# microsoft/AI2BMD

Hardware: NVIDIA H100
Metric: MD steps/sec (higher is better)
Workload: dtype f32

## Files before the change

### ai2bmd_b200/csrc/engine.cu

```cuda
#include <cuda_runtime.h>

#include <algorithm>
#include <cstdarg>
#include <cstdio>
#include <cstdlib>
#include <cstring>
#include <mutex>
#include <string>
#include <vector>

#include "../../include/visnet_b200.h"
#include "k_edge.cuh"
#include "k_caph.cuh"
#include "k_comm.cuh"
#include "k_edge_tc.cuh"
#include "k_graph_embed.cuh"
#include <nvtx3/nvToolsExt.h>
#include "k_head.cuh"
#include "k_md.cuh"
#include "k_nonbonded.cuh"
#include "k_node.cuh"
#include "k_node2.cuh"
#include "k_node_tc.cuh"

// ... 321 lines not shown
        if (status == cudaSuccess && e != cudaSuccess) status = e;
    }
};

template <int NPW>
void launch_head(Launcher& Lc) {
    vb_handle* h = Lc.h;
    const int blocks = (h->ws.N + NODE_WARPS * NPW - 1) / (NODE_WARPS * NPW);
    Lc.launch(head_kernel<NPW>, dim3(blocks), dim3(NODE_WARPS * 32), HeadSmem<NPW>::BYTES, h->mw, h->ws);
    Lc.check();
}
template <int TE, int NW>
void launch_edge_fwd(Launcher& Lc, int l, int occ) {
    vb_handle* h = Lc.h;
    EdgeArgs a{l, h->mw, h->ws};
    const int tiles = (h->ws.Ecap + TE - 1) / TE;
    const int blocks = std::max(1, std::min(tiles, h->sm_count * occ));
    Lc.launch(edge_fwd_kernel<TE, NW>, dim3(blocks), dim3(NW * 32), edge_fwd_smem_bytes<TE>(), a);
    Lc.check();
}
template <int TE, int NW>
void launch_edge_bwd(Launcher& Lc, int l, int occ) {
    vb_handle* h = Lc.h;
    EdgeArgs a{l, h->mw, h->ws};
    const int tiles = (h->ws.Ecap + TE - 1) / TE;
    const int blocks = std::max(1, std::min(tiles, h->sm_count * occ));
    Lc.launch(edge_bwd_kernel<TE, NW>, dim3(blocks), dim3(NW * 32), edge_bwd_smem_bytes<TE>(), a);
    Lc.check();
}

template <int NB>
void launch_node_fwd2(Launcher& Lc, int k) {
    vb_handle* h = Lc.h;
    NodeArgs a{k, h->mw, h->ws, h->timeline ? h->d_tl + (size_t)2 * L * TC_TL_SLOTS + (size_t)k * N2_TL_SLOTS : nullptr, h->krot};
    Lc.launch(node_fwd2_kernel<NB>, dim3((h->ws.N + NB - 1) / NB), dim3(N2Cfg<NB>::THREADS), sizeof(NodeFwd2Smem<NB>), a);
    Lc.check();
}
template <int NB>
void launch_node_bwd2(Launcher& Lc, int k) {
    vb_handle* h = Lc.h;
    NodeArgs a{k, h->mw, h->ws, h->timeline ? h->d_tl + (size_t)2 * L * TC_TL_SLOTS + (size_t)(L + 1 + k) * N2_TL_SLOTS : nullptr, h->krot};
    Lc.launch(node_bwd2_kernel<NB>, dim3((h->ws.N + NB - 1) / NB), dim3(N2Cfg<NB>::THREADS), sizeof(NodeBwd2Smem<NB>), a);
    Lc.check();
}
int node_nb(const vb_handle* h) {
    if (h->node_nb > 0) return h->node_nb;
    for (int nb = 1; nb <= 4; nb++)
        if ((h->ws.N + nb - 1) / nb <= h->sm_count) return nb;
    return 8;
}
void node_fwd(Launcher& Lc, int k) {
    if (Lc.h->npw == 2) launch_node_fwd2<16>(Lc, k);
    else switch (node_nb(Lc.h)) {
        case 1: launch_node_fwd2<1>(Lc, k); break;
        case 2: launch_node_fwd2<2>(Lc, k); break;
        case 3: launch_node_fwd2<3>(Lc, k); break;
        case 4: launch_node_fwd2<4>(Lc, k); break;
        default: launch_node_fwd2<8>(Lc, k);
    }
}
void node_bwd(Launcher& Lc, int k) {
    switch (node_nb(Lc.h)) {
        case 1: launch_node_bwd2<1>(Lc, k); break;
        case 2: launch_node_bwd2<2>(Lc, k); break;
        case 3: launch_node_bwd2<3>(Lc, k); break;
        case 4: launch_node_bwd2<4>(Lc, k); break;
        default: launch_node_bwd2<8>(Lc, k);
    }
}
void head(Launcher& Lc) {
    vb_handle* h = Lc.h;
    if (h->ws.N <= 4096) {
        Lc.launch(head2_kernel, dim3(h->ws.N), dim3(128), 0, h->mw, h->ws);
        Lc.check();
        return;
    }
    h->npw == 2 ? launch_head<2>(Lc) : launch_head<1>(Lc);
}
void launch_edge_fwd_tc(Launcher& Lc, int l) {
    vb_handle* h = Lc.h;
    EdgeTcArgs a{};
    a.layer = l; a.mw = h->mw; a.ws = h->ws;
    const LayerW& lw = h->mw.layer[l];
    const size_t chunk = 4 * 8192;
    int n = 0;
    a.jobs[n++] = TcJob{lw.tcW1, 0};
    a.jobs[n++] = TcJob{lw.tcW1 + chunk, 0};
    if (l < L - 1) a.jobs[n++] = TcJob{lw.tcW1 + 2 * chunk, 0};
    a.jobs[n++] = TcJob{lw.tcWs, 0};
    a.jobs[n++] = TcJob{lw.tcWs + chunk, 0};
    a.njobs = n;
    a.tl = h->timeline ? h->d_tl + (size_t)l * TC_TL_SLOTS : nullptr;
    a.tile_rows = h->tile_rows;
    const int rows = h->tc_rows;
    const int tiles = (h->ws.Ecap + h->tile_rows - 1) / h->tile_rows;
    const int blocks = std::max(1, std::min(tiles, h->sm_count));
    if (rows == 32) Lc.launch(edge_fwd_tc_kernel<32>, dim3(blocks), dim3(TC2_THREADS), TC_SMEM_BYTES, a);
    else if (rows == 64) Lc.launch(edge_fwd_tc_kernel<64>, dim3(blocks), dim3(TC2_THREADS), TC_SMEM_BYTES, a);
    else if (rows == 96) Lc.launch(edge_fwd_tc_kernel<96>, dim3(blocks), dim3(TC2_THREADS), TC_SMEM_BYTES, a);
    else Lc.launch(edge_fwd_tc_kernel<128>, dim3(blocks), dim3(TC2_THREADS), TC_SMEM_BYTES, a);
    Lc.check();
}

void edge_fwd(Launcher& Lc, int l) {
    if (Lc.h->edge_tc & 1) { launch_edge_fwd_tc(Lc, l); return; }
    if (Lc.h->te_fwd == 64) launch_edge_fwd<64, 8>(Lc, l, 2);
    else launch_edge_fwd<32, 8>(Lc, l, 4);
}
void launch_edge_bwd_tc(Launcher& Lc, int l) {
    vb_handle* h = Lc.h;
    EdgeTcArgs a{};
    a.layer = l; a.mw = h->mw; a.ws = h->ws;
    const LayerW& lw = h->mw.layer[l];
    const size_t chunk = 4 * 8192;
    const bool upd = l < L - 1;
    int n = 0;
    a.jobs[n++] = TcJob{lw.tcWsN, 0};
    a.jobs[n++] = TcJob{lw.tcWsN + chunk, 1};
    a.jobs[n++] = TcJob{lw.tcW1N + chunk, 0};
    a.jobs[n++] = TcJob{lw.tcW1N, 1};
    if (upd) a.jobs[n++] = TcJob{lw.tcW1N + 2 * chunk, 1};
    a.njobs = n;
    a.tl = h->timeline ? h->d_tl + (size_t)(L + l) * TC_TL_SLOTS : nullptr;
    a.tile_rows = h->tile_rows;
    const int rows = h->tc_rows;
    const int tiles = (h->ws.Ecap + h->tile_rows - 1) / h->tile_rows;
    const int blocks = std::max(1, std::min(tiles, h->sm_count));
    if (rows == 32) Lc.launch(edge_bwd_tc_kernel<32>, dim3(blocks), dim3(TC2_THREADS), TC_SMEM_BYTES, a);
    else if (rows == 64) Lc.launch(edge_bwd_tc_kernel<64>, dim3(blocks), dim3(TC2_THREADS), TC_SMEM_BYTES, a);
    else if (rows == 96) Lc.launch(edge_bwd_tc_kernel<96>, dim3(blocks), dim3(TC2_THREADS), TC_SMEM_BYTES, a);
    else Lc.launch(edge_bwd_tc_kernel<128>, dim3(blocks), dim3(TC2_THREADS), TC_SMEM_BYTES, a);
    Lc.check();
}

void edge_bwd(Launcher& Lc, int l) {
    if (Lc.h->edge_tc & 2) { launch_edge_bwd_tc(Lc, l); return; }
    if (Lc.h->te_bwd == 64) launch_edge_bwd<64, 8>(Lc, l, 1);
    else launch_edge_bwd<32, 8>(Lc, l, 2);
}

void node_tc_common(const vb_handle* h, NodeTcArgs& a, int k) {
    a.layer = k; a.mw = h->mw; a.ws = h->ws;
    a.tx = (h->ws.N + TC_TE - 1) / TC_TE;
    a.tv = (3 * h->ws.N + TC_TE - 1) / TC_TE;
    a.njx = 3; a.njv = 5; a.jx = 1; a.jv = 1;
}
void node_tc_jobs(TcJob* jobs, const float* img, int n) {
    for (int c = 0; c < n; c++) jobs[c] = TcJob{img + (size_t)c * 4 * 8192, 0};
}
int node_tc_grid(const NodeTcArgs& a) { return a.tx * (a.njx / a.jx) + a.tv * (a.njv / a.jv); }
bool node_tc_split(const vb_handle* h, const NodeTcArgs&) { return h->ws.gxa_parts == 3; }

void launch_node_oproj_tc(Launcher& Lc, int k) {
    vb_handle* h = Lc.h;
    NodeTcArgs a{};
    node_tc_common(h, a, k);
    a.tv = 0;
    node_tc_jobs(a.jobs_x, h->mw.layer[k - 1].tcWo, 3);
    if (!node_tc_split(h, a)) a.jx = 3;
    Lc.launch(node_tc_kernel<NT_OPROJ>, dim3(node_tc_grid(a)), dim3(TC2_THREADS), TC_SMEM_BYTES, a);
    Lc.check();
}
void launch_node_norm_fwd(Launcher& Lc, int k) {
    vb_handle* h = Lc.h;
    Lc.launch(node_norm_fwd_kernel, dim3((h->ws.N + NN_WARPS - 1) / NN_WARPS), dim3(NN_WARPS * 32), 0, k, h->mw, h->ws);
    Lc.check();
}
void launch_node_proj_tc(Launcher& Lc, int k) {
    vb_handle* h = Lc.h;
    NodeTcArgs a{};
    node_tc_common(h, a, k);
    node_tc_jobs(a.jobs_x, h->mw.layer[k].tcWqkv, 3);
    node_tc_jobs(a.jobs_v, h->mw.layer[k].tcWvt, 5);
    if (k == 0) a.tv = 0;
    if (k == L - 1) a.njv = 3;
    if (!node_tc_split(h, a)) { a.jx = a.njx; a.jv = a.njv; }
    Lc.launch(node_tc_kernel<NT_PROJ>, dim3(node_tc_grid(a)), dim3(TC2_THREADS), TC_SMEM_BYTES, a);
    Lc.check();
}
void launch_node_bwdA_tc(Launcher& Lc, int k) {
    vb_handle* h = Lc.h;
    NodeTcArgs a{};
    node_tc_common(h, a, k);
    node_tc_jobs(a.jobs_x, h->mw.layer[k].tcWqkvN, 3);
    node_tc_jobs(a.jobs_v, h->mw.layer[k].tcWvtN, 5);
    if (k == L - 1) a.njv = 3;
    a.acc_qkv = h->ws.GQKV; a.acc_tu = h->ws.GTU;
    if (!node_tc_split(h, a)) { a.jx = a.njx; a.jv = a.njv; }
    Lc.launch(node_tc_kernel<NT_BWDA>, dim3(node_tc_grid(a)), dim3(TC2_THREADS), TC_SMEM_BYTES, a);
    Lc.check();
}
void launch_node_norm_bwd(Launcher& Lc, int k) {
    vb_handle* h = Lc.h;
    NodeTcArgs a{};
    node_tc_common(h, a, k);
    if (k == L - 1) a.njv = 3;
    Lc.launch(node_norm_bwd_kernel, dim3((h->ws.N + NN_WARPS - 1) / NN_WARPS), dim3(NN_WARPS * 32), 0, k, h->mw, h->ws,
              h->ws.GQKV, h->ws.GVNMSG, h->ws.GTU, node_tc_split(h, a) ? 1 : 0);
    Lc.check();
}
void launch_node_bwdB_tc(Launcher& Lc, int k) {
    vb_handle* h = Lc.h;
    NodeTcArgs a{};
    node_tc_common(h, a, k);
    a.tv = 0;
    node_tc_jobs(a.jobs_x, h->mw.layer[k - 1].tcWoN, 3);
    if (h->ws.gxa_parts == 1) a.jx = 3;
    Lc.launch(node_tc_kernel<NT_BWDB>, dim3(node_tc_grid(a)), dim3(TC2_THREADS), TC_SMEM_BYTES, a);
    Lc.check();
}
void node_fwd_tc(Launcher& Lc, int k) {
    char name[64];
    if (k >= 1) { snprintf(name, sizeof(name), "oproj%d", k); if (Lc.next(name)) launch_node_oproj_tc(Lc, k); }
    snprintf(name, sizeof(name), "norm%d", k);
    if (Lc.next(name)) launch_node_norm_fwd(Lc, k);
    if (k < L) { snprintf(name, sizeof(name), "proj%d", k); if (Lc.next(name)) launch_node_proj_tc(Lc, k); }
}
void node_bwd_tc(Launcher& Lc, int k) {
    char name[64];
    if (k <= L - 1) { snprintf(name, sizeof(name), "bwdA%d", k); if (Lc.next(name)) launch_node_bwdA_tc(Lc, k); }
    snprintf(name, sizeof(name), "bnorm%d", k);
    if (Lc.next(name)) launch_node_norm_bwd(Lc, k);
    if (k >= 1) { snprintf(name, sizeof(name), "bwdB%d", k); if (Lc.next(name)) launch_node_bwdB_tc(Lc, k); }
}

void enqueue_finalize(Launcher& Lc, const StepIO& io) {
    vb_handle* h = Lc.h;
    const Workspace& ws = h->ws;
    const bool prot = io.ef != nullptr;
    const int fb = (ws.G + FIN_THREADS / 32 - 1) / (FIN_THREADS / 32);
    const int pb = prot ? (h->n_protein + FIN_THREADS - 1) / FIN_THREADS : 0;
// ... 966 lines not shown
    if (k == "caph_ready") return h->caph_ready ? 1 : 0;
    if (k == "caph_evals") {
        int v = 0;
        if (!h->caph_ready || cudaDeviceSynchronize() != cudaSuccess ||
            cudaMemcpy(&v, h->caph.evals_out, sizeof(int), cudaMemcpyDeviceToHost) != cudaSuccess) return VB_ERR_STATE;
        return v;
    }
    if (k == "comm_ready") return h->comm_ready ? 1 : 0;
    if (k == "edge_overflow") {
        int flag = 0;
        if (h->d_flags && cudaMemcpy(&flag, h->d_flags, sizeof(int), cudaMemcpyDeviceToHost) != cudaSuccess) return VB_ERR_CUDA;
        return flag;
    }
    if (k == "timeline") return h->timeline;
    if (k == "tc_rows") return h->tc_rows;
    if (k == "tile_rows") return h->tile_rows;
    if (k == "n_edges_capacity") return h->ws.Ecap;
    return VB_ERR_ARG;
}

int vb_num_stages(const vb_handle* h) { return h ? (int)h->stage_names.size() : 0; }
const char* vb_stage_name(const vb_handle* h, int stage) {
    if (!h || stage < 0 || stage >= (int)h->stage_names.size()) return "";
    return h->stage_names[stage].c_str();
}

int vb_debug_run(vb_handle* h, const float* pos_dev, int n_stages) {
    if (!h) return VB_ERR_ARG;
    std::lock_guard<std::mutex> lk(h->mu);
    if (!h->has_topology || !pos_dev) { h->set_error("vb_debug_run: bad state/arguments"); return VB_ERR_STATE; }
    CUDA_TRY(h, cudaSetDevice(h->device));
    CUDA_TRY(h, cudaMemcpy(h->d_pos, pos_dev, sizeof(float) * 3 * h->ws.N, cudaMemcpyDeviceToDevice));
    if (h->accum_dirty) { if (int rc = clean_accumulators(h, h->own_stream)) return rc; }
    Launcher Lc{h, h->own_stream, n_stages, 0, false};
    enqueue_all(Lc, internal_io(h, h->n_protein > 0));
    if (Lc.status != cudaSuccess) { h->set_error("debug launch failed: %s", cudaGetErrorString(Lc.status)); return VB_ERR_CUDA; }
    CUDA_TRY(h, cudaStreamSynchronize(h->own_stream));
    h->accum_dirty = n_stages >= 0 && n_stages < (int)h->stage_names.size();
    return VB_OK;
}

int vb_profile_stages(vb_handle* h, const float* pos_dev, int n_iter, float* ms_per_stage_host) {
    if (!h) return VB_ERR_ARG;
    std::lock_guard<std::mutex> lk(h->mu);
    if (!h->has_topology || !pos_dev || !ms_per_stage_host || n_iter <= 0) { h->set_error("vb_profile_stages: bad state/arguments"); return VB_ERR_STATE; }
    CUDA_TRY(h, cudaSetDevice(h->device));
    const int ns = (int)h->stage_names.size();
    std::vector<cudaEvent_t> ev(ns + 1);
    for (auto& e : ev) CUDA_TRY(h, cudaEventCreate(&e));
    std::vector<double> acc(ns, 0.0);
    CUDA_TRY(h, cudaMemcpy(h->d_pos, pos_dev, sizeof(float) * 3 * h->ws.N, cudaMemcpyDeviceToDevice));
    int rc = VB_OK;
    for (int it = 0; it < n_iter + 1 && rc == VB_OK; it++) {
        Launcher Lc{h, h->own_stream, -1, 0, false};
        Lc.events = &ev;
        enqueue_all(Lc, internal_io(h, h->n_protein > 0));
        cudaEventRecord(ev[ns], h->own_stream);
        if (Lc.status != cudaSuccess || cudaStreamSynchronize(h->own_stream) != cudaSuccess) {
            h->set_error("vb_profile_stages: launch failed: %s", cudaGetErrorString(cudaGetLastError()));
            rc = VB_ERR_CUDA;
            break;
        }
        if (it == 0) continue;
        for (int s = 0; s < ns; s++) {
            float ms = 0.f;
            cudaEventElapsedTime(&ms, ev[s], ev[s + 1]);
            acc[s] += ms;
        }
    }
    for (auto& e : ev) cudaEventDestroy(e);
    if (rc == VB_OK)
        for (int s = 0; s < ns; s++) ms_per_stage_host[s] = (float)(acc[s] / n_iter);
    return rc;
}

int vb_tc_selftest(int device, const float* a_host, const float* img_host, float* d_host, int reps, float* ms_out) {
    return vb_tc_selftest_rows(device, TC_TE, a_host, img_host, d_host, reps, ms_out);
}

int vb_tc_selftest_rows(int device, int rows, const float* a_host, const float* img_host, float* d_host, int reps, float* ms_out) {
    if (!a_host || !img_host || !d_host || reps <= 0 || (rows != 32 && rows != 64 && rows != TC_TE)) return VB_ERR_ARG;
    if (cudaSetDevice(device) != cudaSuccess) { g_create_error = "vb_tc_selftest: cudaSetDevice failed"; return VB_ERR_CUDA; }
    float *dA = nullptr, *dI = nullptr, *dD = nullptr;
    const size_t nA = (size_t)TC_TE * D * sizeof(float), nI = (size_t)(D / tc::SLAB_K) * tc::STAGE_BYTES;
    cudaMalloc(&dA, nA); cudaMalloc(&dI, nI); cudaMalloc(&dD, nA);
    cudaMemcpy(dA, a_host, nA, cudaMemcpyHostToDevice);
    cudaMemcpy(dI, img_host, nI, cudaMemcpyHostToDevice);
    cudaMemset(dD, 0, nA);
    void (*kernel)(const float*, const float*, float*, int) =
        rows == 32 ? tc_selftest_kernel<32> : rows == 64 ? tc_selftest_kernel<64> : tc_selftest_kernel<TC_TE>;
    cudaFuncSetAttribute(kernel, cudaFuncAttributeMaxDynamicSharedMemorySize, (int)TC_SMEM_BYTES);
    cudaEvent_t e0, e1;
    cudaEventCreate(&e0); cudaEventCreate(&e1);
    cudaEventRecord(e0);
    kernel<<<1, TC2_THREADS, TC_SMEM_BYTES>>>(dA, dI, dD, reps);
    cudaEventRecord(e1);
    cudaError_t err = cudaDeviceSynchronize();
    float ms = 0.f;
    cudaEventElapsedTime(&ms, e0, e1);
    if (ms_out) *ms_out = ms;
    if (err == cudaSuccess) err = cudaMemcpy(d_host, dD, nA, cudaMemcpyDeviceToHost);
    cudaFree(dA); cudaFree(dI); cudaFree(dD);
    cudaEventDestroy(e0); cudaEventDestroy(e1);
    if (err != cudaSuccess) { g_create_error = std::string("vb_tc_selftest: ") + cudaGetErrorString(err); return VB_ERR_CUDA; }
    return VB_OK;
}

int64_t vb_debug_read(vb_handle* h, const char* name, int layer, void* host_dst, int64_t cap_bytes) {
    if (!h || !name || !host_dst) return VB_ERR_ARG;
    std::lock_guard<std::mutex> lk(h->mu);
    if (!h->has_topology) return VB_ERR_STATE;
    const Workspace& ws = h->ws;
    const size_t N = ws.N, E = ws.Ecap, G = ws.G;
    const void* src = nullptr;
    size_t bytes = 0;
    const std::string k(name);
    auto lay = [&](int hi) { return layer >= 0 && layer < hi; };
#define BUF(key, ptr, count, elt) if (k == key) { src = (ptr); bytes = (size_t)(count) * (elt); }
    if (k == "X" && lay(L + 1)) { src = ws.X[layer]; bytes = N * D * 4; }
    else if (k == "V" && lay(L + 1)) { src = ws.V[layer]; bytes = N * 3 * D * 4; }
    else if (k == "F" && lay(L)) { src = ws.F[layer]; bytes = E * D * 4; }
    else if (k == "VN" && lay(L)) { src = ws.VN[layer]; bytes = N * 3 * D * 4; }
    else if (k == "QKV" && lay(L)) { src = ws.QKV[layer]; bytes = N * 3 * D * 4; }
    else if (k == "V123" && lay(L)) { src = ws.V123[layer]; bytes = N * 9 * D * 4; }
    else if (k == "VDOT" && lay(L)) { src = ws.VDOT[layer]; bytes = N * D * 4; }
    else if (k == "TU" && lay(L)) { src = ws.TU[layer]; bytes = N * 6 * D * 4; }
    else if (k == "O" && lay(L)) { src = ws.O[layer]; bytes = N * 3 * D * 4; }
    else if (k == "P1" && lay(L)) { src = ws.P1[layer]; bytes = E * 3 * D * 4; }
    else if (k == "SP" && lay(L)) { src = ws.SP[layer]; bytes = E * 2 * D * 4; }
    else if (k == "ATT" && lay(L)) { src = ws.ATT[layer]; bytes = E * H * 4; }
    else if (k == "TL" && lay(2 * L) && h->d_tl) { src = h->d_tl + (size_t)layer * TC_TL_SLOTS; bytes = TC_TL_SLOTS * 8; }
    else if (k == "TLN" && lay(2 * L + 3) && h->d_tl) { src = h->d_tl + (size_t)2 * L * TC_TL_SLOTS + (size_t)layer * N2_TL_SLOTS; bytes = N2_TL_SLOTS * 8; }
    else BUF("XA", ws.XA, N * D, 4)
    else BUF("VA", ws.VA, N * 3 * D, 4)
    else BUF("GX", ws.GX, N * D, 4)
    else BUF("GVEC", ws.GVEC, N * 3 * D, 4)
    else BUF("GF", ws.GF, E * D, 4)
    else BUF("GXA", ws.GXA, N * D, 4)
    else BUF("GXA3", ws.GXA, 3 * N * D, 4)
    else BUF("GQKV", ws.GQKV, N * 3 * D, 4)
    else BUF("GVNMSG", ws.GVNMSG, N * 3 * D, 4)
    else BUF("GTU", ws.GTU, N * 6 * D, 4)
    else BUF("geom", ws.geom, E * 8, 4)
    else BUF("rbf", ws.rbf, E * NR, 4)
    else BUF("eacc", ws.eacc, E * 4, 4)
    else BUF("grbf", ws.grbf, E * NR, 4)
    else BUF("esrc", ws.esrc, E, 4)
    else BUF("edst", ws.edst, E, 4)
    else BUF("rowptr", ws.rowptr, N + 1, 4)
    else BUF("eatom", ws.eatom, N, 4)
    else BUF("energy", h->d_energy, G, 4)
    else BUF("forces", h->d_forces, N * 3, 4)
#undef BUF
    if (!src) { h->set_error("vb_debug_read: unknown buffer %s[%d]", name, layer); return VB_ERR_ARG; }
    if ((int64_t)bytes > cap_bytes) bytes = (size_t)cap_bytes;
    if (cudaSetDevice(h->device) != cudaSuccess || cudaDeviceSynchronize() != cudaSuccess ||
        cudaMemcpy(host_dst, src, bytes, cudaMemcpyDeviceToHost) != cudaSuccess) {
        h->set_error("vb_debug_read: copy failed: %s", cudaGetErrorString(cudaGetLastError()));
        return VB_ERR_CUDA;
    }
    return (int64_t)bytes;
}

}
```

### ai2bmd_b200/csrc/k_edge_tc.cuh

```cuda
#pragma once
#include "k_edge.cuh"
#include "tc_common.cuh"

namespace vb {

constexpr int TC_TE = 128;
constexpr int TC_STAGES = 2;
constexpr int TC_MAX_STAGES = 3;
constexpr int TC_SLABS = D / tc::SLAB_K;
static_assert((TC_SLABS & (TC_SLABS - 1)) == 0, "tc_slab rotates the slab order with a mask: TC_SLABS must be a power of two");
constexpr int TC_MAXJOBS = 12;
constexpr int TC_LT = D + LDS_PAD;

struct TcJob {
    const float* img;
    int accumulate;
};

struct TcShared {
    alignas(1024) uint8_t ring[TC_STAGES][tc::STAGE_BYTES];
    alignas(16) float tile[TC_TE][TC_LT];
    alignas(16) float abuf[TC_TE][TC_LT];
    EdgeMeta<TC_TE> meta;
    alignas(8) uint64_t b_full[TC_MAX_STAGES];
    uint64_t b_tile;
    uint32_t released[TC_MAX_STAGES];
    const TcJob* jobs;
    int njobs, nslabs;
    alignas(16) float eacc[TC_TE][4];
    float gattn[TC_TE][H];
};

__device__ __forceinline__ TcShared* tc_shared_base(uint8_t* raw) {
    const uint32_t s = tc::smem_u32(raw);
    return reinterpret_cast<TcShared*>(raw + (((s + 1023u) & ~1023u) - s));
}
constexpr size_t TC_SMEM_BYTES = sizeof(TcShared) + 1024;
static_assert(TC_SMEM_BYTES <= 227 * 1024, "tensor-core kernels must fit the 227 KB of shared memory of an H100 block");

__host__ __device__ constexpr int tc_nstages(int rows) { return rows <= 64 ? 3 : 2; }
constexpr size_t TC_STAGE2_OFF = offsetof(TcShared, abuf) + sizeof(float) * 64 * TC_LT;
static_assert(TC_STAGE2_OFF % 1024 == 0 && sizeof(float) * (TC_TE - 64) * TC_LT >= tc::STAGE_BYTES,
              "the third ring stage must fit the upper half of abuf on a swizzle-atom boundary");
__device__ __forceinline__ uint8_t* tc_stage_ptr(TcShared& sh, int stage) {
    return stage < TC_STAGES ? sh.ring[stage] : reinterpret_cast<uint8_t*>(&sh.abuf[64][0]);
}

__device__ __forceinline__ int tc_slab(int s) { return (s + (int)blockIdx.x) & (TC_SLABS - 1); }

template <int NS>
__device__ __forceinline__ void tc_issue(TcShared& sh, int k) {
    if (k >= sh.nslabs) return;
    const int stage = k % NS, job = (k / TC_SLABS) % sh.njobs, s = tc_slab(k % TC_SLABS);
    const char* src = reinterpret_cast<const char*>(sh.jobs[job].img) + (size_t)s * tc::STAGE_BYTES;
    tc::mbar_arrive_expect_tx(&sh.b_full[stage], tc::STAGE_BYTES);
    tc::tma_load_1d(tc_stage_ptr(sh, stage), src, tc::STAGE_BYTES, &sh.b_full[stage]);
}

}


namespace vb {

constexpr int TC2_CWARPS = 16;
constexpr int TC2_CTHREADS = TC2_CWARPS * 32;
constexpr int TC2_THREADS = TC2_CTHREADS;
constexpr int TC2_NGRP = TC2_CTHREADS / D;

struct EdgeTcArgs {
    int layer;
    ModelW mw;
    Workspace ws;
    TcJob jobs[TC_MAXJOBS];
    int njobs;
    int tile_rows;
    unsigned long long* tl;
};
constexpr int TC_TL_SLOTS = 64;
#define TC_TL(k) do { if (a.tl != nullptr && blockIdx.x == 0 && it == 0 && threadIdx.x == 0) a.tl[k] = (unsigned long long)clock64(); } while (0)

__device__ __forceinline__ void csync() { asm volatile("bar.sync 1, %0;" ::"n"(TC2_CTHREADS) : "memory"); }

template <int ROWS>
struct TcRing {
    static constexpr int NS = tc_nstages(ROWS);
    int next = 0;
};

template <int ROWS>
__device__ __forceinline__ void tc2_setup(TcShared& sh, const TcRing<ROWS>&, const TcJob* jobs, int njobs, int ntiles) {
    constexpr int NS = TcRing<ROWS>::NS;
    if (threadIdx.x == 0) {
        for (int s = 0; s < NS; s++) { tc::mbar_init(&sh.b_full[s], 1); sh.released[s] = 0; }
        tc::mbar_init(&sh.b_tile, TC2_CWARPS);
        sh.jobs = jobs; sh.njobs = njobs; sh.nslabs = ntiles * njobs * TC_SLABS;
        tc::fence_barrier_init();
    }
    __syncthreads();
    if (threadIdx.x == 0)
        for (int k = 0; k < NS; k++) tc_issue<NS>(sh, k);
}

template <int NS>
__device__ __forceinline__ void tc2_release(TcShared& sh, int k, int lane) {
    __syncwarp();
    if (lane == 0) {
        const uint32_t before = tc::atom_add_acq_rel(&sh.released[k % NS], 1u);
        if (before % TC2_CWARPS == TC2_CWARPS - 1) tc_issue<NS>(sh, k + NS);
    }
}

__device__ __forceinline__ void tc2_tile_to_a(TcShared& sh, int rows) {
    csync();
    for (int idx = threadIdx.x; idx < rows * (D / 4); idx += TC2_CTHREADS) {
        const int r = idx >> 5, c = (idx & 31) * 4;
        st4(&sh.abuf[r][c], ld4(&sh.tile[r][c]));
    }
}

template <int ROWS>
__device__ __forceinline__ void tc2_mma(TcShared& sh, TcRing<ROWS>& ring, float (&acc)[32], int accumulate, int warp, int lane,
                                        int nvalid) {
    constexpr int NS = TcRing<ROWS>::NS;
    csync();
    const int q = warp >> 2, m0 = (q & 1) * 64 + (warp & 3) * 16, g = lane >> 2, t = lane & 3;
    const bool active = (q & 1) * 64 < nvalid;
    if (!accumulate) {
#pragma unroll
        for (int i = 0; i < 32; i++) acc[i] = 0.f;
    }
#pragma unroll 1
    for (int s = 0; s < TC_SLABS; s++) {
        const int k = ring.next + s, stage = k % NS;
        if (active) {
            uint32_t ahi[4][4], alo[4][4];
            const int k0 = tc_slab(s) * tc::SLAB_K + t;
#pragma unroll
            for (int kk = 0; kk < 4; kk++) {
                const int kc = k0 + kk * 8;
                tc::split_tf32(sh.abuf[m0 + g][kc], ahi[kk][0], alo[kk][0]);
                tc::split_tf32(sh.abuf[m0 + g + 8][kc], ahi[kk][1], alo[kk][1]);
                tc::split_tf32(sh.abuf[m0 + g][kc + 4], ahi[kk][2], alo[kk][2]);
                tc::split_tf32(sh.abuf[m0 + g + 8][kc + 4], ahi[kk][3], alo[kk][3]);
            }
            tc::mbar_wait(&sh.b_full[stage], (uint32_t)(k / NS) & 1u);
            const uint32_t bhi = tc::smem_u32(tc_stage_ptr(sh, stage)) + (uint32_t)(q >> 1) * (64 * 128);
            const uint32_t blo = bhi + tc::SLAB_BYTES;
            tc::wgmma_fence();
#pragma unroll
            for (int kk = 0; kk < 4; kk++) {
                const uint64_t dhi = tc::smem_desc_sw128(bhi + kk * 32);
                const uint64_t dlo = tc::smem_desc_sw128(blo + kk * 32);
                tc::mma_m64n64k8_tf32(acc, alo[kk], dhi);
                tc::mma_m64n64k8_tf32(acc, ahi[kk], dlo);
                tc::mma_m64n64k8_tf32(acc, ahi[kk], dhi);
            }
            tc::wgmma_commit();
            tc::wgmma_wait_all();
#pragma unroll
            for (int kk = 0; kk < 4; kk++)
#pragma unroll
                for (int i = 0; i < 4; i++) { tc::reg_fence(ahi[kk][i]); tc::reg_fence(alo[kk][i]); }
#pragma unroll
            for (int i = 0; i < 32; i++) tc::reg_fence(acc[i]);
        } else {
            tc::mbar_wait(&sh.b_full[stage], (uint32_t)(k / NS) & 1u);
        }
        tc2_release<NS>(sh, k, lane);
    }
    ring.next += TC_SLABS;
}

__device__ __forceinline__ void tc2_acc_to_tile(TcShared& sh, const float (&acc)[32], int warp, int lane, int nvalid) {
    const int q = warp >> 2, r = (q & 1) * 64 + (warp & 3) * 16 + (lane >> 2), c = (q >> 1) * 64 + 2 * (lane & 3);
#pragma unroll
    for (int i = 0; i < 8; i++) {
        if (r < nvalid) *reinterpret_cast<float2*>(&sh.tile[r][c + 8 * i]) = make_float2(acc[4 * i], acc[4 * i + 1]);
        if (r + 8 < nvalid) *reinterpret_cast<float2*>(&sh.tile[r + 8][c + 8 * i]) = make_float2(acc[4 * i + 2], acc[4 * i + 3]);
    }
}

template <int ROWS>
__global__ void __launch_bounds__(TC2_THREADS, 1) tc_selftest_kernel(const float* __restrict__ A, const float* __restrict__ img,
                                                                     float* __restrict__ Dout, int reps) {
    extern __shared__ __align__(1024) uint8_t dyn_raw[];
    TcShared& sh = *tc_shared_base(dyn_raw);
    __shared__ TcJob jobs[1];
    if (threadIdx.x == 0) jobs[0] = TcJob{img, 0};
    TcRing<ROWS> ring;
    tc2_setup(sh, ring, jobs, 1, reps);
    const int warp = threadIdx.x >> 5, lane = threadIdx.x & 31;
    float acc[32];
    for (int t = 0; t < reps; t++) {
        for (int idx = threadIdx.x; idx < ROWS * (D / 4); idx += TC2_CTHREADS) {
            const int r = idx >> 5, c = (idx & 31) * 4;
            st4(&sh.tile[r][c], ld4(A + (size_t)r * D + c));
        }
        tc2_tile_to_a(sh, ROWS);
        tc2_mma(sh, ring, acc, 0, warp, lane, ROWS);
        csync();
        tc2_acc_to_tile(sh, acc, warp, lane, ROWS);
        csync();
        for (int idx = threadIdx.x; idx < ROWS * (D / 4); idx += TC2_CTHREADS) {
            const int r = idx >> 5, c = (idx & 31) * 4;
            st4(Dout + (size_t)r * D + c, ld4(&sh.tile[r][c]));
        }
        csync();
    }
}

template <int ROWS>
__global__ void __launch_bounds__(TC2_THREADS, 1) edge_fwd_tc_kernel(const __grid_constant__ EdgeTcArgs a) {
    pdl_entry();
    extern __shared__ __align__(1024) uint8_t dyn_raw[];
    TcShared& sh = *tc_shared_base(dyn_raw);
    const Workspace& ws = a.ws;
    const int l = a.layer;
    const LayerW& lw = a.mw.layer[l];
    const bool upd = (l < L - 1);
    const int J_DK = 0, J_DV = 1, J_F = 2, J_S1 = upd ? 3 : 2, J_S2 = upd ? 4 : 3;
    constexpr int RPW = ROWS / TC2_CWARPS;
    const int warp = threadIdx.x >> 5, lane = threadIdx.x & 31, col = lane * 4;
    const int E = ws.rowptr[ws.N];
    const int trows = min(ROWS, max(16, a.tile_rows));
    const int ntiles_total = (E + trows - 1) / trows;
    const int my_tiles = ((int)blockIdx.x < ntiles_total) ? (ntiles_total - (int)blockIdx.x + (int)gridDim.x - 1) / (int)gridDim.x : 0;
    if (a.tl != nullptr && blockIdx.x == 0 && threadIdx.x == 0) a.tl[0] = (unsigned long long)clock64();
    TcRing<ROWS> ring;
// ... 562 lines not shown
```

### ai2bmd_b200/csrc/model.h

```cpp
#pragma once
#include <cuda_runtime.h>
#include <stddef.h>
#include "common.cuh"

namespace vb {

#define VB_GLOBAL_WEIGHTS(X)                                                                      \
    X(emb, 100 * D)                \
    X(nb_emb, 100 * D)             \
    X(rbf_means, NR) X(rbf_betas, NR)                                                              \
    X(WdN, D * NR) X(WdT, NR * D) X(bd, D)      \
    X(WcT, 2 * D * D) X(bc, D) X(WcN, D * 2 * D)         \
    X(WeN, D * NR) X(WeT, NR * D) X(be, D)              \
    X(on_w, D) X(on_b, D) X(von_w, D)          \
    X(h0_W1T, D * D) X(h0_W1N, D * D)                  \
    X(h0_W2T, D * 64) X(h0_W2N, 64 * D)                \
    X(h0_U0T, 2 * D * D) X(h0_b0, D) X(h0_U0N, D * 2 * D)         \
    X(h0_U2T, D * D) X(h0_b2, D) X(h0_U2N, D * D)                 \
    X(h1_W1T, 64 * 64) X(h1_W1N, 64 * 64)              \
    X(h1_U0T, D * 64) X(h1_b0, 64) X(h1_U0N, 64 * D)              \
    X(h1_u2, 64) X(h1_b2, 4)                        \
    X(atomref, 100) X(scalars, 4)

#define VB_LAYER_WEIGHTS(X)                                                                       \
    X(ln_w, D) X(ln_b, D) X(vln_w, D)                                                              \
    X(WqkvT, D * 3 * D) X(bqkv, 3 * D) X(WqkvN, 3 * D * D)           \
    X(WvecT, D * 3 * D) X(WvecN, 3 * D * D)                          \
    X(WtuT, D * 2 * D) X(WtuN, 2 * D * D)                     \
    X(W1T, D * 3 * D) X(b1, 3 * D) X(W1N, 3 * D * D)          \
    X(WsT, D * 2 * D) X(bs, 2 * D) X(WsN, 2 * D * D)                 \
    X(WoT, D * 3 * D) X(bo, 3 * D) X(WoN, 3 * D * D)                 \
     \
    X(tcW1, 3 * 4 * 8192)              \
    X(tcWs, 2 * 4 * 8192)              \
    X(tcWsN, 2 * 4 * 8192)             \
    X(tcW1N, 3 * 4 * 8192)             \
                     \
    X(tcWo, 3 * 4 * 8192)              \
    X(tcWqkv, 3 * 4 * 8192)            \
    X(tcWvt, 5 * 4 * 8192)      \
    X(tcWoN, 3 * 4 * 8192)             \
    X(tcWqkvN, 3 * 4 * 8192)           \
    X(tcWvtN, 5 * 4 * 8192)

struct LayerW {
#define X(name, count) const float* name;
    VB_LAYER_WEIGHTS(X)
#undef X
};

struct ModelW {
#define X(name, count) const float* name;
    VB_GLOBAL_WEIGHTS(X)
#undef X
    LayerW layer[L];
    float cutoff;
};

struct Workspace {
    int N, G, Ecap;
    const int* z;
    const int* frag_of;
    const int* frag_start;
    int* deg;
    int* slots;
    int* rowptr;
    int* esrc;
    int* edst;
    float* geom;
    float* rbf;
    float* eacc;
    float* grbf;
    float* X[L + 1];
    float* V[L + 1];
    float* F[L];
    float* VN[L];
    float* QKV[L];
    float* V123[L];
    float* VDOT[L];
    float* TU[L];
    float* O[L];
    float* P1[L];
    float* SP[L];
    float* ATT[L];
    float* XA;
    float* VA;
    float* GX;
    float* GVEC;
    float* GF;
    float* GXA;
    int gxa_parts;
    float* GQKV;
    float* GVNMSG;
    float* GTU;
    float* eatom;
    float* XN;
    float* PX;
    float* PV;
    float* GO;
};

__device__ __forceinline__ float4 load_gxa(const Workspace& ws, size_t node, int col) {
    float4 v = ld4(ws.GXA + node * D + col);
    if (ws.gxa_parts == 3) v = (v + ld4(ws.GXA + ((size_t)ws.N + node) * D + col)) + ld4(ws.GXA + (2 * (size_t)ws.N + node) * D + col);
    return v;
}

}
```

### ai2bmd_b200/csrc/tc_common.cuh

```cuda
#pragma once
#include <cuda_runtime.h>
#include <stdint.h>

namespace vb {
namespace tc {

__device__ __forceinline__ uint32_t smem_u32(const void* p) { return (uint32_t)__cvta_generic_to_shared(p); }

__device__ __forceinline__ void mbar_init(uint64_t* bar, uint32_t count) {
    asm volatile("mbarrier.init.shared::cta.b64 [%0], %1;" ::"r"(smem_u32(bar)), "r"(count));
}
__device__ __forceinline__ void fence_barrier_init() { asm volatile("fence.mbarrier_init.release.cluster;" ::: "memory"); }
__device__ __forceinline__ void mbar_arrive(uint64_t* bar) {
    asm volatile("{\n\t.reg .b64 st;\n\tmbarrier.arrive.shared::cta.b64 st, [%0];\n\t}" ::"r"(smem_u32(bar)) : "memory");
}
__device__ __forceinline__ void mbar_arrive_expect_tx(uint64_t* bar, uint32_t bytes) {
    asm volatile("{\n\t.reg .b64 st;\n\tmbarrier.arrive.expect_tx.shared::cta.b64 st, [%0], %1;\n\t}" ::"r"(smem_u32(bar)),
                 "r"(bytes)
                 : "memory");
}
__device__ __forceinline__ uint32_t atom_add_acq_rel(uint32_t* p, uint32_t v) {
    uint32_t old;
    asm volatile("atom.acq_rel.cta.shared::cta.add.u32 %0, [%1], %2;" : "=r"(old) : "r"(smem_u32(p)), "r"(v) : "memory");
    return old;
}
__device__ __forceinline__ void mbar_wait(uint64_t* bar, uint32_t parity) {
    asm volatile(
        "{\n\t"
        ".reg .pred p;\n\t"
        "WAIT_LOOP:\n\t"
        "mbarrier.try_wait.parity.shared::cta.b64 p, [%0], %1;\n\t"
        "@p bra WAIT_DONE;\n\t"
        "bra WAIT_LOOP;\n\t"
        "WAIT_DONE:\n\t"
        "}" ::"r"(smem_u32(bar)),
        "r"(parity)
        : "memory");
}

__device__ __forceinline__ void tma_load_1d(void* smem_dst, const void* gmem_src, uint32_t bytes, uint64_t* bar) {
    asm volatile("cp.async.bulk.shared::cluster.global.mbarrier::complete_tx::bytes [%0], [%1], %2, [%3];" ::"r"(
                     smem_u32(smem_dst)),
                 "l"(gmem_src), "r"(bytes), "r"(smem_u32(bar))
                 : "memory");
}

__device__ __forceinline__ void tma_prefetch_l2(const void* gmem_src, uint32_t bytes) {
    asm volatile("cp.async.bulk.prefetch.L2.global [%0], %1;" ::"l"(gmem_src), "r"(bytes) : "memory");
}

__device__ __forceinline__ uint64_t smem_desc_sw128(uint32_t saddr) {
    return (uint64_t)((saddr & 0x3FFFFu) >> 4) | (1ull << 16) | (64ull << 32) | (1ull << 62);
}
__device__ __forceinline__ void wgmma_fence() { asm volatile("wgmma.fence.sync.aligned;" ::: "memory"); }
__device__ __forceinline__ void wgmma_commit() { asm volatile("wgmma.commit_group.sync.aligned;" ::: "memory"); }
__device__ __forceinline__ void wgmma_wait_all() { asm volatile("wgmma.wait_group.sync.aligned 0;" ::: "memory"); }
__device__ __forceinline__ void reg_fence(uint32_t& r) { asm volatile("" : "+r"(r)::"memory"); }
__device__ __forceinline__ void reg_fence(float& r) { asm volatile("" : "+f"(r)::"memory"); }

__device__ __forceinline__ void mma_m64n64k8_tf32(float (&d)[32], const uint32_t (&a)[4], uint64_t desc_b) {
    asm volatile(
        "{\n\t"
        "wgmma.mma_async.sync.aligned.m64n64k8.f32.tf32.tf32 "
        "{%0,%1,%2,%3,%4,%5,%6,%7,%8,%9,%10,%11,%12,%13,%14,%15,"
        "%16,%17,%18,%19,%20,%21,%22,%23,%24,%25,%26,%27,%28,%29,%30,%31}, "
        "{%32,%33,%34,%35}, %36, 1, 1, 1;\n\t"
        "}"
        : "+f"(d[0]), "+f"(d[1]), "+f"(d[2]), "+f"(d[3]), "+f"(d[4]), "+f"(d[5]), "+f"(d[6]), "+f"(d[7]), "+f"(d[8]),
          "+f"(d[9]), "+f"(d[10]), "+f"(d[11]), "+f"(d[12]), "+f"(d[13]), "+f"(d[14]), "+f"(d[15]), "+f"(d[16]),
          "+f"(d[17]), "+f"(d[18]), "+f"(d[19]), "+f"(d[20]), "+f"(d[21]), "+f"(d[22]), "+f"(d[23]), "+f"(d[24]),
          "+f"(d[25]), "+f"(d[26]), "+f"(d[27]), "+f"(d[28]), "+f"(d[29]), "+f"(d[30]), "+f"(d[31])
        : "r"(a[0]), "r"(a[1]), "r"(a[2]), "r"(a[3]), "l"(desc_b)
        : "memory");
}

__device__ __forceinline__ void split_tf32(float x, uint32_t& hi, uint32_t& lo) {
    asm("cvt.rna.tf32.f32 %0, %1;" : "=r"(hi) : "f"(x));
    const float rest = x - __uint_as_float(hi);
    asm("cvt.rna.tf32.f32 %0, %1;" : "=r"(lo) : "f"(rest));
}

constexpr int SLAB_K = 32;
constexpr int SLAB_BYTES = 128 * SLAB_K * 4;
constexpr int STAGE_BYTES = 2 * SLAB_BYTES;

}
}
```

### ai2bmd_b200/weights.py

```python
from __future__ import annotations

import re
from typing import Dict

import numpy as np

D, L = 128, 6


def load_state_dict(path: str) -> Dict[str, np.ndarray]:
    if path.endswith(".npz"):
        z = np.load(path)
        return {k: np.asarray(z[k], dtype=np.float32) for k in z.files}
    import torch
    try:
        ck = torch.load(path, map_location="cpu", weights_only=True)
    except Exception as e:
        raise RuntimeError(f"{path}: torch.load(weights_only=True) refused the file ({e}); the reference loads it with full "
                           "unpickling -- for a TRUSTED file, re-save its state_dict (or an .npz of it) and load that") from e
    hp = ck.get("hyper_parameters", {})
    if hp:
        want = dict(embedding_dimension=128, num_layers=6, num_heads=8, num_rbf=32, lmax=1, max_num_neighbors=32,
                    vecnorm_type="max_min", rbf_type="expnorm", activation="silu", attn_activation="silu", cutoff=5.0,
                    max_z=100, prior_model="Atomref", reduce_op="add", derivative=True)
# ... 13 lines not shown
    out["rbf_means"] = f(rm + "distance_expansion.means")
    out["rbf_betas"] = f(rm + "distance_expansion.betas")
    out["WdN"] = f(rm + "neighbor_embedding.distance_proj.weight")
    out["WdT"] = out["WdN"].T
    out["bd"] = f(rm + "neighbor_embedding.distance_proj.bias")
    wc = f(rm + "neighbor_embedding.combine.weight")
    out["WcT"], out["bc"], out["WcN"] = wc.T, f(rm + "neighbor_embedding.combine.bias"), wc
    out["WeN"] = f(rm + "edge_embedding.edge_proj.weight")
    out["WeT"] = out["WeN"].T
    out["be"] = f(rm + "edge_embedding.edge_proj.bias")
    out["on_w"], out["on_b"] = f(rm + "out_norm.weight"), f(rm + "out_norm.bias")
    out["von_w"] = f(rm + "vec_out_norm.weight")
    for tag, pre in (("h0", o0), ("h1", o1)):
        w1 = f(pre + "vec1_proj.weight")
        out[f"{tag}_W1T"], out[f"{tag}_W1N"] = w1.T, w1
        u0 = f(pre + "update_net.0.weight")
        out[f"{tag}_U0T"], out[f"{tag}_b0"], out[f"{tag}_U0N"] = u0.T, f(pre + "update_net.0.bias"), u0
    w2 = f(o0 + "vec2_proj.weight")
    out["h0_W2T"], out["h0_W2N"] = w2.T, w2
    u2 = f(o0 + "update_net.2.weight")
    out["h0_U2T"], out["h0_b2"], out["h0_U2N"] = u2.T, f(o0 + "update_net.2.bias"), u2
    out["h1_u2"] = f(o1 + "update_net.2.weight")[0]
    out["h1_b2"] = np.array([f(o1 + "update_net.2.bias")[0], 0, 0, 0], dtype=np.float32)
    out["atomref"] = (f("prior_model.atomref.weight").reshape(-1) if "prior_model.atomref.weight" in sd
                      else np.zeros(100, dtype=np.float32))
    out["scalars"] = np.array([float(sd.get("std", 1.0)), float(sd.get("mean", 0.0)), 0, 0], dtype=np.float32)
    for l in range(L):
        p = rm + f"vis_mp_layers.{l}."
        last = l == L - 1
        z = np.zeros((D, D), dtype=np.float32)
        zb = np.zeros((D,), dtype=np.float32)
        k = f"layer{l}."
        out[k + "ln_w"], out[k + "ln_b"] = f(p + "layernorm.weight"), f(p + "layernorm.bias")
        out[k + "vln_w"] = f(p + "vec_layernorm.weight")
        wqkv = np.concatenate([f(p + "q_proj.weight"), f(p + "k_proj.weight"), f(p + "v_proj.weight")], 0)
        out[k + "WqkvT"], out[k + "WqkvN"] = wqkv.T, wqkv
        out[k + "bqkv"] = np.concatenate([f(p + "q_proj.bias"), f(p + "k_proj.bias"), f(p + "v_proj.bias")])
        wv = f(p + "vec_proj.weight")
        out[k + "WvecT"], out[k + "WvecN"] = wv.T, wv
        wtu = np.concatenate([z if last else f(p + "w_trg_proj.weight"), z if last else f(p + "w_src_proj.weight")], 0)
        out[k + "WtuT"], out[k + "WtuN"] = wtu.T, wtu
        w1 = np.concatenate([f(p + "dk_proj.weight"), f(p + "dv_proj.weight"), z if last else f(p + "f_proj.weight")], 0)
        out[k + "W1T"], out[k + "W1N"] = w1.T, w1
        out[k + "b1"] = np.concatenate([f(p + "dk_proj.bias"), f(p + "dv_proj.bias"), zb if last else f(p + "f_proj.bias")])
        ws = f(p + "s_proj.weight")
        out[k + "WsT"], out[k + "bs"], out[k + "WsN"] = ws.T, f(p + "s_proj.bias"), ws
        wo = f(p + "o_proj.weight")
        out[k + "WoT"], out[k + "bo"], out[k + "WoN"] = wo.T, f(p + "o_proj.bias"), wo
        out[k + "tcW1"] = np.concatenate([tc_image(w1[c * D:(c + 1) * D]) for c in range(3)])
        out[k + "tcWs"] = np.concatenate([tc_image(ws[c * D:(c + 1) * D]) for c in range(2)])
        out[k + "tcWsN"] = np.concatenate([tc_image(ws[c * D:(c + 1) * D].T) for c in range(2)])
        out[k + "tcW1N"] = np.concatenate([tc_image(w1[c * D:(c + 1) * D].T) for c in range(3)])
        wvt = np.concatenate([wv, wtu], 0)
        out[k + "tcWo"] = np.concatenate([tc_image(wo[c * D:(c + 1) * D]) for c in range(3)])
        out[k + "tcWqkv"] = np.concatenate([tc_image(wqkv[c * D:(c + 1) * D]) for c in range(3)])
        out[k + "tcWvt"] = np.concatenate([tc_image(wvt[c * D:(c + 1) * D]) for c in range(5)])
        out[k + "tcWoN"] = np.concatenate([tc_image(wo[c * D:(c + 1) * D].T) for c in range(3)])
        out[k + "tcWqkvN"] = np.concatenate([tc_image(wqkv[c * D:(c + 1) * D].T) for c in range(3)])
        out[k + "tcWvtN"] = np.concatenate([tc_image(wvt[c * D:(c + 1) * D].T) for c in range(5)])
    return out


def pack_weights(sd: Dict[str, np.ndarray], manifest: str) -> np.ndarray:
    arrays = _named_arrays(sd)
    parts = []
    for item in manifest.strip(";").split(";"):
        name, count = item.split(":")
        a = np.ascontiguousarray(arrays[name], dtype=np.float32).reshape(-1)
        if a.size != int(count):
            raise ValueError(f"weight {name}: have {a.size} values, manifest wants {count}")
        parts.append(a)
    return np.concatenate(parts)


def round_tf32(x: np.ndarray) -> np.ndarray:
    b = np.ascontiguousarray(x, dtype=np.float32).view(np.uint32)
    return ((b + np.uint32(0x1000)) & np.uint32(0xFFFFE000)).view(np.float32)


def tc_image(w_nk: np.ndarray) -> np.ndarray:
    w = np.ascontiguousarray(w_nk, dtype=np.float32)
    n, k = w.shape
    assert n == 128 and k % 32 == 0
    hi = round_tf32(w)
    lo = round_tf32(w - hi)
    rows = np.arange(128)
    out = np.empty((k // 32, 2, 128, 8, 4), dtype=np.float32)
    for s in range(k // 32):
        for p, plane in enumerate((hi, lo)):
            blk = plane[:, s * 32:(s + 1) * 32].reshape(128, 8, 4)
            for c in range(8):
                out[s, p, rows, c ^ (rows & 7), :] = blk[:, c, :]
    return out.reshape(-1)
```

Baseline: 1047.

## Store single-plane fp32 weight images and split hi/lo TF32 in shared memory

Weight images for the TC kernels now hold raw fp32 values instead of precomputed hi/lo TF32 planes, which halves the bytes TMA must load per slab. After each slab lands, the kernel splits it into hi and lo planes in shared memory. For small row tiles, idle warps do the split ahead of time and signal new split mbarriers. Otherwise the active warps split inline and sync on named barriers. This trades global and L2 traffic for extra split ALU work, proxy fences and added synchronisation in the pipeline.

Measured after the change: 1064, median of 6. 1.02x the previous value.

```diff
diff --git a/ai2bmd_b200/csrc/engine.cu b/ai2bmd_b200/csrc/engine.cu
--- a/ai2bmd_b200/csrc/engine.cu
+++ b/ai2bmd_b200/csrc/engine.cu
@@ -427,7 +427,7 @@
     EdgeTcArgs a{};
     a.layer = l; a.mw = h->mw; a.ws = h->ws;
     const LayerW& lw = h->mw.layer[l];
-    const size_t chunk = 4 * 8192;
+    const size_t chunk = tc::CHUNK_FLOATS;
     int n = 0;
     a.jobs[n++] = TcJob{lw.tcW1, 0};
     a.jobs[n++] = TcJob{lw.tcW1 + chunk, 0};
@@ -457,7 +457,7 @@
     EdgeTcArgs a{};
     a.layer = l; a.mw = h->mw; a.ws = h->ws;
     const LayerW& lw = h->mw.layer[l];
-    const size_t chunk = 4 * 8192;
+    const size_t chunk = tc::CHUNK_FLOATS;
     const bool upd = l < L - 1;
     int n = 0;
     a.jobs[n++] = TcJob{lw.tcWsN, 0};
@@ -491,7 +491,7 @@
     a.njx = 3; a.njv = 5; a.jx = 1; a.jv = 1;
 }
 void node_tc_jobs(TcJob* jobs, const float* img, int n) {
-    for (int c = 0; c < n; c++) jobs[c] = TcJob{img + (size_t)c * 4 * 8192, 0};
+    for (int c = 0; c < n; c++) jobs[c] = TcJob{img + (size_t)c * tc::CHUNK_FLOATS, 0};
 }
 int node_tc_grid(const NodeTcArgs& a) { return a.tx * (a.njx / a.jx) + a.tv * (a.njv / a.jv); }
 bool node_tc_split(const vb_handle* h, const NodeTcArgs&) { return h->ws.gxa_parts == 3; }
@@ -1624,7 +1624,7 @@
     if (!a_host || !img_host || !d_host || reps <= 0 || (rows != 32 && rows != 64 && rows != TC_TE)) return VB_ERR_ARG;
     if (cudaSetDevice(device) != cudaSuccess) { g_create_error = "vb_tc_selftest: cudaSetDevice failed"; return VB_ERR_CUDA; }
     float *dA = nullptr, *dI = nullptr, *dD = nullptr;
-    const size_t nA = (size_t)TC_TE * D * sizeof(float), nI = (size_t)(D / tc::SLAB_K) * tc::STAGE_BYTES;
+    const size_t nA = (size_t)TC_TE * D * sizeof(float), nI = (size_t)tc::CHUNK_FLOATS * sizeof(float);
     cudaMalloc(&dA, nA); cudaMalloc(&dI, nI); cudaMalloc(&dD, nA);
     cudaMemcpy(dA, a_host, nA, cudaMemcpyHostToDevice);
     cudaMemcpy(dI, img_host, nI, cudaMemcpyHostToDevice);
diff --git a/ai2bmd_b200/csrc/k_edge_tc.cuh b/ai2bmd_b200/csrc/k_edge_tc.cuh
--- a/ai2bmd_b200/csrc/k_edge_tc.cuh
+++ b/ai2bmd_b200/csrc/k_edge_tc.cuh
@@ -23,6 +23,7 @@
     alignas(16) float abuf[TC_TE][TC_LT];
     EdgeMeta<TC_TE> meta;
     alignas(8) uint64_t b_full[TC_MAX_STAGES];
+    uint64_t b_split[TC_MAX_STAGES][2];
     uint64_t b_tile;
     uint32_t released[TC_MAX_STAGES];
     const TcJob* jobs;
@@ -52,9 +53,36 @@
 __device__ __forceinline__ void tc_issue(TcShared& sh, int k) {
     if (k >= sh.nslabs) return;
     const int stage = k % NS, job = (k / TC_SLABS) % sh.njobs, s = tc_slab(k % TC_SLABS);
-    const char* src = reinterpret_cast<const char*>(sh.jobs[job].img) + (size_t)s * tc::STAGE_BYTES;
-    tc::mbar_arrive_expect_tx(&sh.b_full[stage], tc::STAGE_BYTES);
-    tc::tma_load_1d(tc_stage_ptr(sh, stage), src, tc::STAGE_BYTES, &sh.b_full[stage]);
+    const char* src = reinterpret_cast<const char*>(sh.jobs[job].img) + (size_t)s * tc::SLAB_BYTES;
+    tc::mbar_arrive_expect_tx(&sh.b_full[stage], tc::SLAB_BYTES);
+    tc::tma_load_1d(tc_stage_ptr(sh, stage), src, tc::SLAB_BYTES, &sh.b_full[stage]);
+}
+
+template <int NT>
+__device__ __forceinline__ void tc2_split_b(uint8_t* stage, int half, int tid, int nthreads) {
+    constexpr int N4 = tc::SLAB_BYTES / 2 / 16;
+    constexpr int LO4 = tc::SLAB_BYTES / 16;
+    float4* p = reinterpret_cast<float4*>(stage + half * (tc::SLAB_BYTES / 2));
+    auto split4 = [&](int i, const float4 v) {
+        uint4 hi, lo;
+        tc::split_tf32(v.x, hi.x, lo.x);
+        tc::split_tf32(v.y, hi.y, lo.y);
+        tc::split_tf32(v.z, hi.z, lo.z);
+        tc::split_tf32(v.w, hi.w, lo.w);
+        reinterpret_cast<uint4*>(p)[i] = hi;
+        reinterpret_cast<uint4*>(p)[i + LO4] = lo;
+    };
+    if constexpr (NT > 0) {
+        float4 v[N4 / NT];
+#pragma unroll
+        for (int j = 0; j < N4 / NT; j++) v[j] = p[tid + j * NT];
+#pragma unroll
+        for (int j = 0; j < N4 / NT; j++) split4(tid + j * NT, v[j]);
+    } else {
+#pragma unroll 1
+        for (int i = tid; i < N4; i += nthreads) split4(i, p[i]);
+    }
+    tc::fence_proxy_async_smem();
 }
 
 }
@@ -85,13 +113,19 @@
 struct TcRing {
     static constexpr int NS = tc_nstages(ROWS);
     int next = 0;
+    int split = 0;
 };
 
 template <int ROWS>
 __device__ __forceinline__ void tc2_setup(TcShared& sh, const TcRing<ROWS>&, const TcJob* jobs, int njobs, int ntiles) {
     constexpr int NS = TcRing<ROWS>::NS;
     if (threadIdx.x == 0) {
-        for (int s = 0; s < NS; s++) { tc::mbar_init(&sh.b_full[s], 1); sh.released[s] = 0; }
+        for (int s = 0; s < NS; s++) {
+            tc::mbar_init(&sh.b_full[s], 1);
+            tc::mbar_init(&sh.b_split[s][0], 4);
+            tc::mbar_init(&sh.b_split[s][1], 4);
+            sh.released[s] = 0;
+        }
         tc::mbar_init(&sh.b_tile, TC2_CWARPS);
         sh.jobs = jobs; sh.njobs = njobs; sh.nslabs = ntiles * njobs * TC_SLABS;
         tc::fence_barrier_init();
@@ -125,6 +159,23 @@
     csync();
     const int q = warp >> 2, m0 = (q & 1) * 64 + (warp & 3) * 16, g = lane >> 2, t = lane & 3;
     const bool active = (q & 1) * 64 < nvalid;
+    constexpr bool SPLIT_AHEAD = ROWS <= 64;
+    if (SPLIT_AHEAD && !active) {
+        const int end = min(ring.next + TC_SLABS + 1, sh.nslabs);
+#pragma unroll 1
+        for (int k = ring.split; k < end; k++) {
+            const int stage = k % NS;
+            tc::mbar_wait(&sh.b_full[stage], (uint32_t)(k / NS) & 1u);
+            tc2_split_b<128>(tc_stage_ptr(sh, stage), q >> 1, threadIdx.x & 127, 128);
+            __syncwarp();
+            if (lane == 0) tc::mbar_arrive(&sh.b_split[stage][q >> 1]);
+            tc2_release<NS>(sh, k, lane);
+        }
+        ring.split = max(ring.split, end);
+        ring.next += TC_SLABS;
+        return;
+    }
+    const int nsplit = nvalid > 64 ? 256 : 128;
     if (!accumulate) {
 #pragma unroll
         for (int i = 0; i < 32; i++) acc[i] = 0.f;
@@ -133,6 +184,12 @@
     for (int s = 0; s < TC_SLABS; s++) {
         const int k = ring.next + s, stage = k % NS;
         if (active) {
+            if (!SPLIT_AHEAD) {
+                tc::mbar_wait(&sh.b_full[stage], (uint32_t)(k / NS) & 1u);
+                tc2_split_b<0>(tc_stage_ptr(sh, stage), q >> 1, (q & 1) * 128 + (threadIdx.x & 127), nsplit);
+                if (q >> 1) tc::named_bar_sync<3>(nsplit);
+                else tc::named_bar_sync<2>(nsplit);
+            }
             uint32_t ahi[4][4], alo[4][4];
             const int k0 = tc_slab(s) * tc::SLAB_K + t;
 #pragma unroll
@@ -143,7 +200,7 @@
                 tc::split_tf32(sh.abuf[m0 + g][kc + 4], ahi[kk][2], alo[kk][2]);
                 tc::split_tf32(sh.abuf[m0 + g + 8][kc + 4], ahi[kk][3], alo[kk][3]);
             }
-            tc::mbar_wait(&sh.b_full[stage], (uint32_t)(k / NS) & 1u);
+            if (SPLIT_AHEAD) tc::mbar_wait(&sh.b_split[stage][q >> 1], (uint32_t)(k / NS) & 1u);
             const uint32_t bhi = tc::smem_u32(tc_stage_ptr(sh, stage)) + (uint32_t)(q >> 1) * (64 * 128);
             const uint32_t blo = bhi + tc::SLAB_BYTES;
             tc::wgmma_fence();
diff --git a/ai2bmd_b200/csrc/model.h b/ai2bmd_b200/csrc/model.h
--- a/ai2bmd_b200/csrc/model.h
+++ b/ai2bmd_b200/csrc/model.h
@@ -2,6 +2,7 @@
 #include <cuda_runtime.h>
 #include <stddef.h>
 #include "common.cuh"
+#include "tc_common.cuh"
 
 namespace vb {
 
@@ -31,17 +32,17 @@
     X(WsT, D * 2 * D) X(bs, 2 * D) X(WsN, 2 * D * D)                 \
     X(WoT, D * 3 * D) X(bo, 3 * D) X(WoN, 3 * D * D)                 \
      \
-    X(tcW1, 3 * 4 * 8192)              \
-    X(tcWs, 2 * 4 * 8192)              \
-    X(tcWsN, 2 * 4 * 8192)             \
-    X(tcW1N, 3 * 4 * 8192)             \
+    X(tcW1, 3 * tc::CHUNK_FLOATS)         \
+    X(tcWs, 2 * tc::CHUNK_FLOATS)         \
+    X(tcWsN, 2 * tc::CHUNK_FLOATS)         \
+    X(tcW1N, 3 * tc::CHUNK_FLOATS)         \
                      \
-    X(tcWo, 3 * 4 * 8192)              \
-    X(tcWqkv, 3 * 4 * 8192)            \
-    X(tcWvt, 5 * 4 * 8192)      \
-    X(tcWoN, 3 * 4 * 8192)             \
-    X(tcWqkvN, 3 * 4 * 8192)           \
-    X(tcWvtN, 5 * 4 * 8192)
+    X(tcWo, 3 * tc::CHUNK_FLOATS)         \
+    X(tcWqkv, 3 * tc::CHUNK_FLOATS)         \
+    X(tcWvt, 5 * tc::CHUNK_FLOATS)  \
+    X(tcWoN, 3 * tc::CHUNK_FLOATS)         \
+    X(tcWqkvN, 3 * tc::CHUNK_FLOATS)         \
+    X(tcWvtN, 5 * tc::CHUNK_FLOATS)
 
 struct LayerW {
 #define X(name, count) const float* name;
diff --git a/ai2bmd_b200/csrc/tc_common.cuh b/ai2bmd_b200/csrc/tc_common.cuh
--- a/ai2bmd_b200/csrc/tc_common.cuh
+++ b/ai2bmd_b200/csrc/tc_common.cuh
@@ -45,6 +45,13 @@
                  : "memory");
 }
 
+__device__ __forceinline__ void fence_proxy_async_smem() { asm volatile("fence.proxy.async.shared::cta;" ::: "memory"); }
+
+template <int ID>
+__device__ __forceinline__ void named_bar_sync(int nthreads) {
+    asm volatile("bar.sync %0, %1;" ::"n"(ID), "r"(nthreads) : "memory");
+}
+
 __device__ __forceinline__ void tma_prefetch_l2(const void* gmem_src, uint32_t bytes) {
     asm volatile("cp.async.bulk.prefetch.L2.global [%0], %1;" ::"l"(gmem_src), "r"(bytes) : "memory");
 }
@@ -83,6 +90,8 @@
 constexpr int SLAB_K = 32;
 constexpr int SLAB_BYTES = 128 * SLAB_K * 4;
 constexpr int STAGE_BYTES = 2 * SLAB_BYTES;
+constexpr int CHUNK_FLOATS = 128 * 128;
+static_assert(CHUNK_FLOATS * 4 == (128 / SLAB_K) * SLAB_BYTES, "a chunk image is its K-slabs' planes back to back");
 
 }
 }
diff --git a/ai2bmd_b200/weights.py b/ai2bmd_b200/weights.py
--- a/ai2bmd_b200/weights.py
+++ b/ai2bmd_b200/weights.py
@@ -119,13 +119,10 @@
     w = np.ascontiguousarray(w_nk, dtype=np.float32)
     n, k = w.shape
     assert n == 128 and k % 32 == 0
-    hi = round_tf32(w)
-    lo = round_tf32(w - hi)
     rows = np.arange(128)
-    out = np.empty((k // 32, 2, 128, 8, 4), dtype=np.float32)
+    out = np.empty((k // 32, 128, 8, 4), dtype=np.float32)
     for s in range(k // 32):
-        for p, plane in enumerate((hi, lo)):
-            blk = plane[:, s * 32:(s + 1) * 32].reshape(128, 8, 4)
-            for c in range(8):
-                out[s, p, rows, c ^ (rows & 7), :] = blk[:, c, :]
+        blk = w[:, s * 32:(s + 1) * 32].reshape(128, 8, 4)
+        for c in range(8):
+            out[s, rows, c ^ (rows & 7), :] = blk[:, c, :]
     return out.reshape(-1)
```
